# bede/kindel

Measured on NVIDIA H100. Metric: aligned bases/sec through pileup+consensus, higher is better.
Workload: dtype int32

## Files before the change

kindel_b200/csrc/api.cu:

```cuda
#include <atomic>
#include <cstdio>
#include <cstdlib>
#include <cstring>
#include <new>

#include "kdl_common.cuh"
#include "pileup_general.cu"
#include "pileup_simple.cu"
#include "pileup_tile.cu"
#include "pileup_mask.cu"
#include "vote.cu"
#include "assemble.cu"
#include "variants.cu"
#include "select.cu"
#include "primers.cu"
#include "mates.cu"
#include "quality.cu"
#include "amplicons.cu"
#include "normalise.cu"

namespace {

std::atomic<long long> g_launches{0};

inline int grid_for(long long items, int per_block, int cap) {
    long long g = (items + per_block - 1) / per_block;
    if (g < 1) g = 1;
    if (g > cap) g = cap;
    return (int)g;
}

#ifndef KDL_HOST_EMU
constexpr int kMaxDevices = 64;

inline int current_device() {
    int dev = 0;
    if (cudaGetDevice(&dev) != cudaSuccess || dev < 0 || dev >= kMaxDevices) dev = 0;
    return dev;
}

inline int sm_count() {
    static std::atomic<int> cache[kMaxDevices];
    const int dev = current_device();
    int n = cache[dev].load(std::memory_order_relaxed);
    if (n <= 0) {
        if (cudaDeviceGetAttribute(&n, cudaDevAttrMultiProcessorCount, dev) != cudaSuccess || n <= 0) n = 132;
        cache[dev].store(n, std::memory_order_relaxed);
    }
    return n;
}

template <int kFlush, bool kCx>
inline int ensure_tile_smem() {
    static std::atomic<int> done[kMaxDevices];
    const int dev = current_device();
    if (done[dev].load(std::memory_order_acquire)) return KDL_OK;
    if (cudaFuncSetAttribute(kdl::pileup_tile_kernel<kFlush, kCx>, cudaFuncAttributeMaxDynamicSharedMemorySize,
                             (int)sizeof(kdl::TileSmem<kdl::TileCfg<kCx>>)) != cudaSuccess)
        return KDL_ERR_CUDA;
    done[dev].store(1, std::memory_order_release);
    return KDL_OK;
}

inline int check_launch() {
    g_launches.fetch_add(1, std::memory_order_relaxed);
    return cudaGetLastError() == cudaSuccess ? KDL_OK : KDL_ERR_CUDA;
}
#else
inline int sm_count() { return emu::M().sm_count; }

template <int kFlush, bool kCx>
inline int ensure_tile_smem() { return KDL_OK; }

inline int check_launch() {
    g_launches.fetch_add(1, std::memory_order_relaxed);
    return emu::take_launch_error() ? KDL_ERR_CUDA : KDL_OK;
}
#endif

template <int kFlush, bool kCx>
inline int launch_tile(const kdl_batch& b, int32_t* counts, long long n_slots, long long tile_lo, long long n_tiles,
                       int split, int zero_rest, uint32_t* dirty_map, uint32_t map_after, cudaStream_t st) {
    int rc = ensure_tile_smem<kFlush, kCx>();
    if (rc != KDL_OK) return rc;
    const long long units = n_tiles * split, max_grid = (long long)sm_count() * 2;
    const long long grid = units < max_grid ? units : max_grid;
    KDL_LAUNCH((kdl::pileup_tile_kernel<kFlush, kCx>), (unsigned)grid, kdl::W_THREADS,
               sizeof(kdl::TileSmem<kdl::TileCfg<kCx>>), st,
               b, counts, n_slots, b.tile_index, tile_lo, n_tiles, split, zero_rest, dirty_map, map_after);
    return KDL_OK;
}

int validate_batch(const kdl_batch* b) {
    if (!b || b->n_reads < 0 || b->n_contigs < 0 || b->n_hard < 0 || b->n_complex < b->n_hard)
        return KDL_ERR_INVALID_ARG;
    if (b->n_reads > 0 && (!b->ref_start || !b->seq_off || !b->l_seq || !b->seq4 ||
                           !b->contig_read_off || !b->contig_len || !b->contig_slot))
        return KDL_ERR_INVALID_ARG;
    if ((b->n_hard > 0 && !b->hard_idx) || (b->n_complex > 0 && !b->complex_idx)) return KDL_ERR_INVALID_ARG;
    if (b->reach_right < b->max_simple_len || b->reach_left < 0) return KDL_ERR_INVALID_ARG;
    return KDL_OK;
}

}

extern "C" {

int kdl_abi_version(void) { return KDL_ABI_VERSION; }

const char* kdl_status_string(int status) {
    switch (status) {
        case KDL_OK: return "ok";
        case KDL_ERR_INVALID_ARG: return "invalid argument";
        case KDL_ERR_CUDA: return "CUDA error";
        case KDL_ERR_NO_DEVICE: return "no CUDA device";
        case KDL_ERR_INDEX: return "IndexError: read walks off the contig or off its SEQ";
        case KDL_ERR_KEY: return "KeyError: base outside A,C,G,T,N in an M or S op";
        default: return "unknown status";
    }
}

int64_t kdl_launch_count(void) { return g_launches.load(std::memory_order_relaxed); }

int kdl_pileup(const kdl_batch* batch, int32_t* counts, int64_t n_slots, int32_t* ins_events,
               int32_t* err_flag, void* stream) {
    return kdl_pileup_range(batch, counts, n_slots, 0, n_slots, 0, ins_events, err_flag, stream);
}

int kdl_pileup_range(const kdl_batch* batch, int32_t* counts, int64_t n_slots, int64_t slot_lo,
                     int64_t slot_hi, int32_t flags, int32_t* ins_events, int32_t* err_flag, void* stream) {
    return kdl_pileup_range_map(batch, counts, n_slots, slot_lo, slot_hi, flags, nullptr, ins_events, err_flag, stream);
}

int kdl_pileup_range_map(const kdl_batch* batch, int32_t* counts, int64_t n_slots, int64_t slot_lo, int64_t slot_hi,
                         int32_t flags, uint32_t* dirty_map, int32_t* ins_events, int32_t* err_flag, void* stream) {
    int rc = validate_batch(batch);
    if (rc != KDL_OK) return rc;
    if (!counts || !err_flag || n_slots <= 0 || slot_lo < 0 || slot_hi > n_slots || slot_lo > slot_hi ||
        (reinterpret_cast<uintptr_t>(dirty_map) & 15))
        return KDL_ERR_INVALID_ARG;
    const bool tileable = (n_slots % KDL_TILE) == 0 && (slot_lo % KDL_TILE) == 0 && (slot_hi % KDL_TILE) == 0;
    if ((slot_lo & 3) || (slot_hi & 3)) return KDL_ERR_INVALID_ARG;
    cudaStream_t st = (cudaStream_t)stream;
    const int cap = sm_count() * 8;
    const bool has_tile_reads = batch->n_reads > batch->n_hard;
    const bool tiled = has_tile_reads && tileable && batch->reads_sorted && batch->tile_index &&
                       batch->reach_right > 0 && batch->reach_right <= KDL_FAST_MAXLEN + KDL_TILE_MAXREACH;
    const bool fresh = (flags & KDL_PILEUP_FRESH_WEIGHTS) != 0;
    const long long tile_lo = slot_lo / KDL_TILE, n_tiles = (slot_hi - slot_lo) / KDL_TILE;
    int split = 1;
    if (tiled && n_tiles > 0) {
        const long long slots = (long long)sm_count() * 2;
        if (n_tiles < slots) {
            long long want = (slots + n_tiles - 1) / n_tiles;
            const long long deep = batch->n_reads / (n_tiles * 256);
            if (want > deep) want = deep;
            split = (int)(want < 1 ? 1 : (want > 32 ? 32 : want));
        }
        if (const char* ev = getenv("KDL_SPLIT")) { const int v = atoi(ev); if (v >= 1 && v <= 64) split = v; }
    }
    bool cx_by_atomics = (batch->n_complex - batch->n_hard) * 16 < batch->n_reads;
    if (const char* ev = getenv("KDL_CX")) cx_by_atomics = !strcmp(ev, "atomics") ? true : (!strcmp(ev, "pieces") ? false : cx_by_atomics);
    const int zero_in_k1 = (tiled && split == 1 && fresh && n_tiles > 0 && (flags & KDL_PILEUP_ZERO_REST)) ? 1 : 0;
    const int zero_from = (fresh && !(tiled && split == 1)) ? 0 : 5;
    const int zero_to = ((flags & KDL_PILEUP_ZERO_REST) && !zero_in_k1) ? KDL_NCOL : 5;
    const bool zero_pass = zero_to > zero_from && slot_hi > slot_lo;
    const bool k1_stores = tiled && split == 1 && fresh && n_tiles > 0;
    const bool saturate = dirty_map && batch->n_complex > 0 && batch->n_complex * 16 >= batch->n_reads &&
                          (k1_stores || zero_pass);
    uint32_t* mark_map = saturate ? nullptr : dirty_map;
    if (zero_pass) {
        uint32_t* zmap = saturate || (zero_from <= 5 && zero_to == KDL_NCOL) ? dirty_map : nullptr;
        KDL_LAUNCH(kdl::zero_cols_kernel, sm_count() * 4, 256, 0, st, counts, n_slots, zero_from, zero_to, slot_lo,
                   slot_hi, zmap, saturate ? ~0u : 0u);
        if ((rc = check_launch()) != KDL_OK) return rc;
    }
    const uint32_t map_after = saturate && k1_stores ? ~0u : 0u;
    if (batch->n_reads == 0) return KDL_OK;
    if (tiled) {
        if (n_tiles > 0) {
            KDL_LAUNCH(kdl::tile_index_kernel, (unsigned)((n_tiles * 32 + 255) / 256), 256, 0, st, *batch, tile_lo,
                       n_tiles, batch->tile_index);
            if ((rc = check_launch()) != KDL_OK) return rc;
            const bool cx = batch->n_complex > batch->n_hard && !cx_by_atomics;
            if (split > 1) {
                rc = cx ? launch_tile<kdl::F_ATOMIC, true>(*batch, counts, n_slots, tile_lo, n_tiles, split, 0, nullptr, 0, st)
                        : launch_tile<kdl::F_ATOMIC, false>(*batch, counts, n_slots, tile_lo, n_tiles, split, 0, nullptr, 0, st);
            } else if (fresh) {
                rc = cx ? launch_tile<kdl::F_STORE, true>(*batch, counts, n_slots, tile_lo, n_tiles, 1, zero_in_k1, dirty_map,
                                                          map_after, st)
                        : launch_tile<kdl::F_STORE, false>(*batch, counts, n_slots, tile_lo, n_tiles, 1, zero_in_k1, dirty_map,
                                                           map_after, st);
            } else {
                rc = cx ? launch_tile<kdl::F_ADD, true>(*batch, counts, n_slots, tile_lo, n_tiles, 1, 0, nullptr, 0, st)
                        : launch_tile<kdl::F_ADD, false>(*batch, counts, n_slots, tile_lo, n_tiles, 1, 0, nullptr, 0, st);
            }
            if (rc != KDL_OK) return rc;
            if ((rc = check_launch()) != KDL_OK) return rc;
        }
        if (batch->n_complex > batch->n_hard) {
            if (cx_by_atomics)
                KDL_LAUNCH(kdl::pileup_events_kernel<8>, (unsigned)((batch->n_complex + 31) / 32), 256, 0, st,
                           *batch, counts, n_slots, ins_events, 1, mark_map);
            else
                KDL_LAUNCH(kdl::pileup_events_kernel<1>, (unsigned)((batch->n_complex + 255) / 256), 256, 0, st,
                           *batch, counts, n_slots, ins_events, 0, mark_map);
            if ((rc = check_launch()) != KDL_OK) return rc;
        }
        if (batch->n_hard > 0) {
            const int grid = grid_for(batch->n_hard, 8, cap);
            KDL_LAUNCH(kdl::pileup_general_kernel, grid, 256, 0, st, *batch, batch->hard_idx, batch->n_hard, counts,
                       n_slots, ins_events, err_flag, mark_map);
            if ((rc = check_launch()) != KDL_OK) return rc;
        }
    } else {
        if (batch->n_reads > batch->n_complex) {
            const int grid = grid_for(batch->n_reads, 8, cap);
            KDL_LAUNCH(kdl::pileup_simple_atomic_kernel, grid, 256, 0, st, *batch, counts, n_slots, err_flag);
            if ((rc = check_launch()) != KDL_OK) return rc;
        }
        if (batch->n_complex > 0) {
            const int grid = grid_for(batch->n_reads, 8, cap);
            KDL_LAUNCH(kdl::pileup_general_kernel, grid, 256, 0, st, *batch, nullptr, batch->n_reads, counts, n_slots,
                       ins_events, err_flag, mark_map);
            if ((rc = check_launch()) != KDL_OK) return rc;
        }
    }
    return KDL_OK;
}

int kdl_unmask(const kdl_batch* batch, const kdl_qmask* qmask, int32_t* counts, int64_t n_slots, void* stream) {
    int rc = validate_batch(batch);
    if (rc != KDL_OK) return rc;
    if (!qmask || !counts || n_slots <= 0 || qmask->n_reads < 0 || qmask->n_bases < 0 || qmask->n_reads > batch->n_reads)
        return KDL_ERR_INVALID_ARG;
    if (qmask->n_reads == 0) return KDL_OK;
    if (!qmask->read_idx || !qmask->off || !qmask->qpos) return KDL_ERR_INVALID_ARG;
    const long long grid = (qmask->n_reads + kdl::kQThreads - 1) / kdl::kQThreads;
    KDL_LAUNCH(kdl::unmask_kernel, (unsigned)grid, kdl::kQThreads, 0, (cudaStream_t)stream, *batch, *qmask, counts,
               n_slots);
    return check_launch();
}

int kdl_diagnose(const kdl_batch* batch, kdl_diag* diag_dev, void* stream) {
    int rc = validate_batch(batch);
    if (rc != KDL_OK) return rc;
    if (!diag_dev) return KDL_ERR_INVALID_ARG;
    cudaStream_t st = (cudaStream_t)stream;
    KDL_LAUNCH(kdl::diagnose_init_kernel, 1, 1, 0, st, diag_dev);
    if ((rc = check_launch()) != KDL_OK) return rc;
    if (batch->n_hard > 0) {
        const long long grid = (batch->n_hard + 255) / 256;
        KDL_LAUNCH(kdl::diagnose_kernel, (unsigned)grid, 256, 0, st, *batch, diag_dev);
        if ((rc = check_launch()) != KDL_OK) return rc;
    }
    KDL_LAUNCH(kdl::diagnose_final_kernel, 1, 1, 0, st, diag_dev);
    return check_launch();
}

int kdl_vote(const int32_t* counts, int64_t n_slots, int64_t min_depth_ceil, uint8_t* calls,
             void* stream) {
    if (!counts || !calls || n_slots <= 0 || (n_slots & 3)) return KDL_ERR_INVALID_ARG;
    kdl::Peers none;
    none.n = 0;
    const long long quads = n_slots / 4;
    const long long grid = (quads + 255) / 256;
    KDL_LAUNCH(kdl::vote_kernel<false>, (unsigned)grid, 256, 0, (cudaStream_t)stream,
               counts, none, n_slots, 0, n_slots, min_depth_ceil, calls, nullptr, kdl::MajorityVote{});
    return check_launch();
}

static bool valid_threshold(double t) { return t >= 0.0 && t <= 1.0; }

int kdl_vote_iupac(const int32_t* counts, int64_t n_slots, int64_t min_depth_ceil, double threshold, uint8_t* calls,
                   void* stream) {
    if (!counts || !calls || n_slots <= 0 || (n_slots & 3) || !valid_threshold(threshold)) return KDL_ERR_INVALID_ARG;
    kdl::Peers none;
    none.n = 0;
    const long long quads = n_slots / 4;
    const long long grid = (quads + 255) / 256;
    KDL_LAUNCH((kdl::vote_kernel<false, kdl::IupacVote>), (unsigned)grid, 256, 0, (cudaStream_t)stream,
               counts, none, n_slots, 0, n_slots, min_depth_ceil, calls, nullptr, kdl::IupacVote{threshold});
    return check_launch();
}

int kdl_derive(const int32_t* counts, int64_t n_slots, int32_t* out, void* stream) {
    if (!counts || !out || n_slots <= 0) return KDL_ERR_INVALID_ARG;
    const long long grid = (n_slots + 255) / 256;
    KDL_LAUNCH(kdl::derive_kernel, (unsigned)grid, 256, 0, (cudaStream_t)stream, counts, n_slots, out);
    return check_launch();
}

int kdl_vote_peers(const int32_t* const* peer_counts, int32_t n_peers, int64_t n_slots,
                   int64_t slot_lo, int64_t slot_hi, int64_t min_depth_ceil, uint8_t* calls,
                   int32_t* reduced, void* stream) {
    return kdl_vote_peers_sparse(peer_counts, nullptr, nullptr, n_peers, n_slots, slot_lo, slot_hi,
                                 min_depth_ceil, calls, reduced, stream);
}

static int make_exchange(const kdl_exchange* x, kdl::Exchange* e, int64_t n_slots) {
    if (!x || x->n_ranks < 1 || x->n_ranks > 16 || x->rank < 0 || x->rank >= x->n_ranks || !x->counter)
        return KDL_ERR_INVALID_ARG;
    e->peers.n = x->n_ranks;
    e->rank = x->rank;
    e->counter = x->counter;
    for (int p = 0; p < x->n_ranks; ++p) {
        if (!x->tables[p] || !x->calls[p] || !x->ready[p] || !x->done[p]) return KDL_ERR_INVALID_ARG;
        e->peers.tab[p] = x->tables[p];
        e->peers.lo[p] = x->foot_lo[p];
        e->peers.hi[p] = n_slots > 0 && x->foot_hi[p] > n_slots ? n_slots : x->foot_hi[p];
        if ((e->peers.lo[p] & 3) || (e->peers.hi[p] & 3)) return KDL_ERR_INVALID_ARG;
        e->calls[p] = x->calls[p];
        e->ready[p] = x->ready[p];
        e->done[p] = x->done[p];
        e->slice_lo[p] = x->slice_lo[p];
        e->slice_hi[p] = x->slice_hi[p];
        if ((x->slice_lo[p] & 3) || (x->slice_hi[p] & 3) || x->slice_hi[p] < x->slice_lo[p]) return KDL_ERR_INVALID_ARG;
    }
    e->ready_local = x->ready[x->rank];
    e->done_local = x->done[x->rank];
    return KDL_OK;
}

int kdl_exchange_signal(const kdl_exchange* x, int32_t epoch, void* stream) {
    kdl::Exchange e;
    int rc = make_exchange(x, &e, 0);
    if (rc != KDL_OK) return rc;
    KDL_LAUNCH(kdl::exchange_signal_kernel, 1, 32, 0, (cudaStream_t)stream, e, epoch);
    return check_launch();
}

int kdl_exchange_wait(const kdl_exchange* x, int32_t epoch, void* stream) {
    kdl::Exchange e;
    int rc = make_exchange(x, &e, 0);
    if (rc != KDL_OK) return rc;
    dim3 grid((unsigned)(sm_count() * 2 / x->n_ranks + 1), (unsigned)x->n_ranks);
    KDL_LAUNCH(kdl::exchange_gather_kernel, grid, 256, 0, (cudaStream_t)stream, e, epoch);
    return check_launch();
}

extern "C++" template <class Vote>
int exchange_vote(const kdl_exchange* x, int64_t n_slots, int64_t min_depth_ceil, int32_t epoch, Vote vote,
                  void* stream) {
    if (n_slots <= 0 || (n_slots & 3)) return KDL_ERR_INVALID_ARG;
    kdl::Exchange e;
    int rc = make_exchange(x, &e, n_slots);
    if (rc != KDL_OK) return rc;
    if (x->slice_hi[x->rank] > n_slots) return KDL_ERR_INVALID_ARG;
    const long long quads = (x->slice_hi[x->rank] - x->slice_lo[x->rank]) / 4;
    long long grid = (quads + 255) / 256;
    const long long cap = (long long)sm_count() * 8;
    if (grid > cap) grid = cap;
    if (grid < 1) grid = 1;
    KDL_LAUNCH(kdl::vote_exchange_kernel<Vote>, (unsigned)grid, 256, 0, (cudaStream_t)stream, e, n_slots,
               min_depth_ceil, epoch, vote);
    return check_launch();
}

int kdl_exchange_vote(const kdl_exchange* x, int64_t n_slots, int64_t min_depth_ceil, int32_t epoch,
                      void* stream) {
    return exchange_vote(x, n_slots, min_depth_ceil, epoch, kdl::MajorityVote{}, stream);
}

int kdl_exchange_vote_iupac(const kdl_exchange* x, int64_t n_slots, int64_t min_depth_ceil, double threshold,
                            int32_t epoch, void* stream) {
    if (!valid_threshold(threshold)) return KDL_ERR_INVALID_ARG;
    return exchange_vote(x, n_slots, min_depth_ceil, epoch, kdl::IupacVote{threshold}, stream);
}

int kdl_cdr_flags(const int32_t* counts, int64_t n_slots, int64_t slot_lo, int64_t slot_hi,
                  double clip_decay_threshold, uint8_t* flags, uint8_t* bases, void* stream) {
    if (!counts || !flags || !bases || n_slots <= 0 || slot_lo < 0 || slot_hi > n_slots || slot_lo > slot_hi)
        return KDL_ERR_INVALID_ARG;
    if (slot_hi == slot_lo) return KDL_OK;
    const long long grid = (slot_hi - slot_lo + 255) / 256;
    KDL_LAUNCH(kdl::cdr_flags_kernel, (unsigned)grid, 256, 0, (cudaStream_t)stream, counts, n_slots, slot_lo, slot_hi,
               clip_decay_threshold, flags, bases);
    return check_launch();
}

int64_t kdl_assemble_scratch_words(int64_t n_slots) {
    return n_slots < 0 ? 0 : (n_slots + 1 + kdl::A_BLOCK - 1) / kdl::A_BLOCK + 1;
}

int kdl_assemble(const uint8_t* calls, int64_t n_slots, const int64_t* contig_slot, const int32_t* contig_len,
                 int32_t n_contigs, const int64_t* ins_slot, const uint32_t* ins_off, const uint8_t* ins_bytes,
                 int64_t n_ins, uint32_t* block_sums, uint32_t* offsets, uint8_t* out, void* stream) {
    if (!calls || n_slots <= 0 || !contig_slot || !contig_len || n_contigs < 0 || n_ins < 0 || !block_sums || !offsets ||
        !out || (n_ins > 0 && (!ins_slot || !ins_off || !ins_bytes)))
        return KDL_ERR_INVALID_ARG;
    kdl::AssembleArgs a;
    a.calls = calls; a.n_slots = n_slots; a.contig_slot = contig_slot; a.contig_len = contig_len; a.n_contigs = n_contigs;
    a.ins_slot = ins_slot; a.ins_off = ins_off; a.ins_bytes = ins_bytes; a.n_ins = n_ins;
    const long long n_blocks = (n_slots + 1 + kdl::A_BLOCK - 1) / kdl::A_BLOCK;
    cudaStream_t st = (cudaStream_t)stream;
    int rc;
    KDL_LAUNCH(kdl::assemble_sums_kernel, (unsigned)n_blocks, kdl::A_THREADS, 0, st, a, block_sums);
    if ((rc = check_launch()) != KDL_OK) return rc;
    KDL_LAUNCH(kdl::assemble_scan_sums_kernel, 1, kdl::A_THREADS, 0, st, block_sums, n_blocks);
    if ((rc = check_launch()) != KDL_OK) return rc;
    KDL_LAUNCH(kdl::assemble_scatter_kernel, (unsigned)n_blocks, kdl::A_THREADS, 0, st, a, block_sums, offsets, out);
    return check_launch();
}

int kdl_consensus_qual(const int32_t* counts, const uint8_t* calls, int64_t n_slots, uint8_t* qual, void* stream) {
    if (!counts || !calls || !qual || n_slots <= 0 || (n_slots & 3)) return KDL_ERR_INVALID_ARG;
    const long long grid = (n_slots / 4 + 255) / 256;
    KDL_LAUNCH(kdl::consensus_qual_kernel, (unsigned)grid, 256, 0, (cudaStream_t)stream, counts, calls, n_slots, qual);
    return check_launch();
}

int kdl_assemble_qual(const uint32_t* offsets, const uint8_t* qual, int64_t n_slots, const int64_t* ins_slot,
                      const uint8_t* ins_qual, int64_t n_ins, uint8_t* out, void* stream) {
    if (!offsets || !qual || !out || n_slots <= 0 || n_ins < 0 || (n_ins > 0 && (!ins_slot || !ins_qual)))
        return KDL_ERR_INVALID_ARG;
    const long long n_blocks = (n_slots + kdl::A_BLOCK - 1) / kdl::A_BLOCK;
    KDL_LAUNCH(kdl::assemble_qual_kernel, (unsigned)n_blocks, kdl::A_THREADS, 0, (cudaStream_t)stream,
               offsets, qual, n_slots, ins_slot, ins_qual, n_ins, out);
    return check_launch();
}

int64_t kdl_variant_scratch_words(int64_t n_slots) {
    return n_slots < 0 ? 0 : (n_slots + kdl::A_BLOCK - 1) / kdl::A_BLOCK + 1;
}

static int variant_args(const int32_t* counts, int64_t n_slots, const int64_t* contig_slot, const int32_t* contig_len,
                        int32_t n_contigs, int64_t abs_floor, double rel_threshold, kdl::VariantArgs* a) {
    if (!counts || n_slots <= 0 || (n_slots & 3) || n_slots > (int64_t)UINT32_MAX || n_contigs < 0 ||
        (n_contigs > 0 && (!contig_slot || !contig_len)) || abs_floor < -1 || abs_floor > (1LL << 31))
        return KDL_ERR_INVALID_ARG;
    *a = kdl::VariantArgs{};
    a->counts = counts; a->n_slots = n_slots;
    a->layout.contig_slot = contig_slot; a->layout.contig_len = contig_len; a->layout.n_contigs = n_contigs;
    a->abs_floor = abs_floor; a->rel_threshold = rel_threshold;
    return KDL_OK;
}

int kdl_variant_count(const int32_t* counts, int64_t n_slots, const int64_t* contig_slot, const int32_t* contig_len,
                      int32_t n_contigs, int64_t abs_floor, double rel_threshold, uint32_t* block_sums, void* stream) {
    kdl::VariantArgs a;
    int rc = variant_args(counts, n_slots, contig_slot, contig_len, n_contigs, abs_floor, rel_threshold, &a);
    if (rc != KDL_OK) return rc;
    if (!block_sums) return KDL_ERR_INVALID_ARG;
    const long long n_blocks = (n_slots + kdl::A_BLOCK - 1) / kdl::A_BLOCK;
    cudaStream_t st = (cudaStream_t)stream;
    KDL_LAUNCH(kdl::variant_sums_kernel, (unsigned)n_blocks, kdl::A_THREADS, 0, st, a, block_sums);
    if ((rc = check_launch()) != KDL_OK) return rc;
    KDL_LAUNCH(kdl::assemble_scan_sums_kernel, 1, kdl::A_THREADS, 0, st, block_sums, n_blocks);
    return check_launch();
}

int kdl_variant_scatter(const int32_t* counts, int64_t n_slots, const int64_t* contig_slot, const int32_t* contig_len,
                        int32_t n_contigs, int64_t abs_floor, double rel_threshold, const uint32_t* block_sums,
                        int64_t n_sites, int64_t* site_slot, int32_t* site_counts, uint8_t* site_mask, void* stream) {
    kdl::VariantArgs a;
    int rc = variant_args(counts, n_slots, contig_slot, contig_len, n_contigs, abs_floor, rel_threshold, &a);
    if (rc != KDL_OK) return rc;
    if (!block_sums || n_sites < 0 || n_sites > n_slots || (n_sites > 0 && (!site_slot || !site_counts || !site_mask)))
        return KDL_ERR_INVALID_ARG;
    const long long n_blocks = (n_slots + kdl::A_BLOCK - 1) / kdl::A_BLOCK;
    KDL_LAUNCH(kdl::variant_scatter_kernel, (unsigned)n_blocks, kdl::A_THREADS, 0, (cudaStream_t)stream,
               a, block_sums, n_sites, site_slot, site_counts, site_mask);
    return check_launch();
}

static int variant_ref_args(const int32_t* counts, int64_t n_slots, const int64_t* contig_slot,
                            const int32_t* contig_len, int32_t n_contigs, const uint8_t* ref, int64_t abs_floor,
                            double rel_threshold, kdl::RefVariantArgs* a) {
    kdl::VariantArgs v;
    int rc = variant_args(counts, n_slots, contig_slot, contig_len, n_contigs, abs_floor, rel_threshold, &v);
    if (rc != KDL_OK) return rc;
    if (!ref || (reinterpret_cast<uintptr_t>(ref) & 3)) return KDL_ERR_INVALID_ARG;
    *a = kdl::RefVariantArgs{};
    a->counts = counts; a->n_slots = n_slots; a->layout = v.layout; a->ref = ref;
    a->abs_floor = abs_floor; a->rel_threshold = rel_threshold;
    return KDL_OK;
}

int kdl_variant_ref_count(const int32_t* counts, int64_t n_slots, const int64_t* contig_slot, const int32_t* contig_len,
                          int32_t n_contigs, const uint8_t* ref, int64_t abs_floor, double rel_threshold,
                          uint32_t* block_sums, void* stream) {
    kdl::RefVariantArgs a;
    int rc = variant_ref_args(counts, n_slots, contig_slot, contig_len, n_contigs, ref, abs_floor, rel_threshold, &a);
    if (rc != KDL_OK) return rc;
    if (!block_sums) return KDL_ERR_INVALID_ARG;
    const long long n_blocks = (n_slots + kdl::A_BLOCK - 1) / kdl::A_BLOCK;
    cudaStream_t st = (cudaStream_t)stream;
    KDL_LAUNCH(kdl::variant_ref_sums_kernel, (unsigned)n_blocks, kdl::A_THREADS, 0, st, a, block_sums);
    if ((rc = check_launch()) != KDL_OK) return rc;
    KDL_LAUNCH(kdl::assemble_scan_sums_kernel, 1, kdl::A_THREADS, 0, st, block_sums, n_blocks);
    return check_launch();
}

int kdl_variant_ref_scatter(const int32_t* counts, int64_t n_slots, const int64_t* contig_slot,
                            const int32_t* contig_len, int32_t n_contigs, const uint8_t* ref, int64_t abs_floor,
                            double rel_threshold, const uint32_t* block_sums, int64_t n_sites, int64_t* site_slot,
                            int32_t* site_counts, int64_t* site_dpa, uint8_t* site_mask, void* stream) {
    kdl::RefVariantArgs a;
    int rc = variant_ref_args(counts, n_slots, contig_slot, contig_len, n_contigs, ref, abs_floor, rel_threshold, &a);
    if (rc != KDL_OK) return rc;
    if (!block_sums || n_sites < 0 || n_sites > n_slots ||
        (n_sites > 0 && (!site_slot || !site_counts || !site_dpa || !site_mask)))
        return KDL_ERR_INVALID_ARG;
    const long long n_blocks = (n_slots + kdl::A_BLOCK - 1) / kdl::A_BLOCK;
    KDL_LAUNCH(kdl::variant_ref_scatter_kernel, (unsigned)n_blocks, kdl::A_THREADS, 0, (cudaStream_t)stream,
               a, block_sums, n_sites, site_slot, site_counts, site_dpa, site_mask);
    return check_launch();
}

// ... 446 lines not shown
```

kindel_b200/csrc/pileup_general.cu:

```cuda
#include "kdl_common.cuh"

namespace kdl {

__global__ void __launch_bounds__(256)
pileup_general_kernel(kdl_batch b, const uint32_t* __restrict__ list, long long n_list, int32_t* __restrict__ counts,
                      long long n_slots, int32_t* __restrict__ ins_events, int32_t* __restrict__ err_flag,
                      uint32_t* __restrict__ dirty_map = nullptr) {
    const int lane = threadIdx.x & 31;
    const bool marks = dirty_map != nullptr && lane == 0;
    const long long warp0 = ((long long)blockIdx.x * blockDim.x + threadIdx.x) >> 5;
    const long long n_warps = ((long long)gridDim.x * blockDim.x) >> 5;
    bool bad = false;

    for (long long j = warp0; j < n_list; j += n_warps) {
        const long long r = list ? (long long)list[j] : j;
        const uint32_t lraw = (uint32_t)b.l_seq[r];
        if (!(lraw & KDL_COMPLEX)) continue;
        const int c = find_contig(b.contig_read_off, b.n_contigs, r);
        const long long L = b.contig_len[c];
        const long long base = b.contig_slot[c];
        const long long lseq = complex_len(lraw);
        const uint32_t* __restrict__ seq = b.seq4 + (size_t)b.seq_off[r];
        const uint32_t* __restrict__ blk = seq + ((lseq + 7) >> 3);
        const uint32_t c0 = 0, c1 = blk[0];
        const uint32_t* __restrict__ cig = blk + 2;
        long long r_pos = b.ref_start[r];
        long long q_pos = 0;
        uint32_t evt = blk[1];

        for (uint32_t i = c0; i < c1; ++i) {
            const uint32_t cg = cig[i];
            const long long len = cg >> 4;
            const int op = cg & 0xF;
            if (op == 0 || op == 7 || op == 8) {
                for (long long k = lane; k < len; k += 32) {
                    const long long q = q_pos + k;
                    const long long idx = pyindex(r_pos + k, L);
                    if (q >= lseq || idx < 0) { bad = true; continue; }
                    const int col = nib2col(nibble_at(seq, q));
                    if (col < 0) { bad = true; continue; }
                    atomicAdd(counts + (long long)(KDL_W_A + col) * n_slots + base + idx, 1);
                }
                r_pos += len;
                q_pos += len;
            } else if (op == 1) {
                if (marks) mark_dirty_py(dirty_map, KDL_INS, 1, base, r_pos, r_pos + 1, L + 1);
                if (lane == 0) {
                    const long long idx = pyindex(r_pos, L + 1);
                    if (idx < 0) {
                        bad = true;
                    } else {
                        atomicAdd(counts + (long long)KDL_INS * n_slots + base + idx, 1);
                        if (ins_events) {
                            int4 e = make_int4((int)(base + idx), (int)r, (int)q_pos, (int)len);
                            reinterpret_cast<int4*>(ins_events)[evt] = e;
                        }
                    }
                }
                evt += 1;
                q_pos += len;
            } else if (op == 2) {
                if (marks) mark_dirty_py(dirty_map, KDL_DEL, 1, base, r_pos, r_pos + len, L + 1);
                for (long long k = lane; k < len; k += 32) {
                    const long long idx = pyindex(r_pos + k, L + 1);
                    if (idx < 0) { bad = true; continue; }
                    atomicAdd(counts + (long long)KDL_DEL * n_slots + base + idx, 1);
                }
                r_pos += len;
            } else if (op == 4) {
                if (i == c0) {
                    if (marks) {
                        mark_dirty_py(dirty_map, KDL_CLIP_ENDS, 1, base, r_pos, r_pos + 1, L + 1);
                        mark_dirty(dirty_map, KDL_CEW_A, 5, base + (r_pos - len > 0 ? r_pos - len : 0),
                                   base + (r_pos < L ? r_pos : L));
                    }
                    if (lane == 0) {
                        const long long idx = pyindex(r_pos, L + 1);
                        if (idx < 0) bad = true;
                        else atomicAdd(counts + (long long)KDL_CLIP_ENDS * n_slots + base + idx, 1);
                    }
                    for (long long g = lane; g < len; g += 32) {
                        if (g >= lseq) { bad = true; continue; }
                        const long long rel = r_pos - len + g;
                        if (rel < 0) continue;
                        if (rel >= L) { bad = true; continue; }
                        const int col = nib2col(nibble_at(seq, g));
                        if (col < 0) { bad = true; continue; }
                        atomicAdd(counts + (long long)(KDL_CEW_A + col) * n_slots + base + rel, 1);
                    }
                    q_pos += len;
                } else {
                    if (lane == 0) {
                        const long long idx = pyindex(r_pos - 1, L + 1);
                        if (idx < 0) bad = true;
                        else atomicAdd(counts + (long long)KDL_CLIP_STARTS * n_slots + base + idx, 1);
                    }
                    long long n_adv = L - r_pos;
                    n_adv = n_adv < 0 ? 0 : (n_adv > len ? len : n_adv);
                    if (marks) {
                        mark_dirty_py(dirty_map, KDL_CLIP_STARTS, 1, base, r_pos - 1, r_pos, L + 1);
                        mark_dirty_py(dirty_map, KDL_CSW_A, 5, base, r_pos, r_pos + n_adv, L);
                    }
                    for (long long k = lane; k < n_adv; k += 32) {
                        const long long q = q_pos + k;
                        const long long idx = pyindex(r_pos + k, L);
                        if (q >= lseq || idx < 0) { bad = true; continue; }
                        const int col = nib2col(nibble_at(seq, q));
                        if (col < 0) { bad = true; continue; }
                        atomicAdd(counts + (long long)(KDL_CSW_A + col) * n_slots + base + idx, 1);
                    }
                    if (n_adv < len && q_pos + n_adv >= lseq) bad = true;
                    r_pos += n_adv;
                    q_pos += n_adv;
                }
            }
        }
    }
    if (bad) atomicOr(err_flag, 1);
}

template <int kLanes>
__global__ void __launch_bounds__(256)
pileup_events_kernel(kdl_batch b, int32_t* __restrict__ counts, long long n_slots, int32_t* __restrict__ ins_events,
                     int with_m, uint32_t* __restrict__ dirty_map = nullptr) {
    const int lane = (int)(threadIdx.x % kLanes);
    constexpr int kStep = kLanes;
    const long long gtid = (long long)blockIdx.x * blockDim.x + threadIdx.x;
    const long long j = gtid / kLanes;
    if (j >= b.n_complex) return;
    const long long r = (long long)b.complex_idx[j];
    const uint32_t lraw = (uint32_t)b.l_seq[r];
    if ((lraw & (KDL_COMPLEX | KDL_HARD)) != KDL_COMPLEX) return;
    const int c = find_contig(b.contig_read_off, b.n_contigs, r);
    const long long slot0 = b.contig_slot[c];
    int32_t* __restrict__ tab = counts + slot0;
    const uint32_t* __restrict__ seq = b.seq4 + (size_t)b.seq_off[r];
    const uint32_t* __restrict__ blk = seq + (((lraw & KDL_LEN_MASK) + 7) >> 3);
    const int n_ops = (int)blk[0];
    uint32_t evt = blk[1];
    const uint32_t* __restrict__ ops = blk + 2;
    long long r_pos = b.ref_start[r];
    int q_pos = 0;
    const bool marks = dirty_map != nullptr && lane == 0;
    for (int o = 0; o < n_ops; ++o) {
        const uint32_t cg = ops[o];
        const int len = (int)(cg >> 4);
        const int op = (int)(cg & 0xF);
        if (op == 0 || op == 7 || op == 8) {
            if (with_m)
                for (int d = lane; d < len; d += kStep)
                    atomicAdd(tab + (long long)(KDL_W_A + nib2col(nibble_at(seq, q_pos + d))) * n_slots + r_pos + d, 1);
            r_pos += len;
            q_pos += len;
        } else if (op == 1) {
            if (lane == 0) {
                if (marks) mark_dirty(dirty_map, KDL_INS, 1, slot0 + r_pos, slot0 + r_pos + 1);
                atomicAdd(tab + (long long)KDL_INS * n_slots + r_pos, 1);
                if (ins_events)
                    reinterpret_cast<int4*>(ins_events)[evt] = make_int4((int)(slot0 + r_pos), (int)r, q_pos, len);
            }
            evt += 1;
            q_pos += len;
        } else if (op == 2) {
            if (marks) mark_dirty(dirty_map, KDL_DEL, 1, slot0 + r_pos, slot0 + r_pos + len);
            for (int d = lane; d < len; d += kStep) atomicAdd(tab + (long long)KDL_DEL * n_slots + r_pos + d, 1);
            r_pos += len;
        } else if (op == 4) {
            if (o == 0) {
                if (marks) {
                    mark_dirty(dirty_map, KDL_CLIP_ENDS, 1, slot0 + r_pos, slot0 + r_pos + 1);
                    mark_dirty(dirty_map, KDL_CEW_A, 5, slot0 + (r_pos - len > 0 ? r_pos - len : 0), slot0 + r_pos);
                }
                if (lane == 0) atomicAdd(tab + (long long)KDL_CLIP_ENDS * n_slots + r_pos, 1);
                for (int g = lane; g < len; g += kStep) {
                    const long long rel = r_pos - len + g;
                    if (rel >= 0) atomicAdd(tab + (long long)(KDL_CEW_A + nib2col(nibble_at(seq, g))) * n_slots + rel, 1);
                }
                q_pos += len;
            } else {
                if (marks) {
                    mark_dirty(dirty_map, KDL_CLIP_STARTS, 1, slot0 + r_pos - 1, slot0 + r_pos);
                    mark_dirty(dirty_map, KDL_CSW_A, 5, slot0 + r_pos, slot0 + r_pos + len);
                }
                if (lane == 0) atomicAdd(tab + (long long)KDL_CLIP_STARTS * n_slots + r_pos - 1, 1);
                for (int d = lane; d < len; d += kStep)
                    atomicAdd(tab + (long long)(KDL_CSW_A + nib2col(nibble_at(seq, q_pos + d))) * n_slots + r_pos + d, 1);
                r_pos += len;
                q_pos += len;
            }
        }
    }
}

__device__ unsigned long long diagnose_read(const kdl_batch& b, long long j) {
    const long long r = (long long)b.hard_idx[j];
    const int c = find_contig(b.contig_read_off, b.n_contigs, r);
    const long long L = b.contig_len[c];
    const long long lseq = complex_len((uint32_t)b.l_seq[r]);
    const uint32_t* __restrict__ seq = b.seq4 + (size_t)b.seq_off[r];
    const uint32_t* __restrict__ blk = seq + ((lseq + 7) >> 3);
    const uint32_t c0 = 0, c1 = blk[0];
    const uint32_t* __restrict__ cig = blk + 2;
    long long r_pos = b.ref_start[r], q_pos = 0;
#define KDL_FAIL(kind, nib)                                                                     \
    return ((unsigned long long)r << 24) | ((unsigned long long)(kind) << 20) |                 \
           ((unsigned long long)(nib) << 16) | (unsigned long long)((i - c0) > 0xFFFF ? 0xFFFF : (i - c0))
    for (uint32_t i = c0; i < c1; ++i) {
        const uint32_t cg = cig[i];
        const long long len = cg >> 4;
        const int op = cg & 0xF;
        if (op == 0 || op == 7 || op == 8) {
            for (long long k = 0; k < len; ++k) {
                if (q_pos >= lseq) KDL_FAIL(0, 0);
                if (pyindex(r_pos, L) < 0) KDL_FAIL(0, 0);
                const int nib = nibble_at(seq, q_pos);
                if (nib2col(nib) < 0) KDL_FAIL(1, nib);
                ++r_pos; ++q_pos;
            }
        } else if (op == 1) {
            if (pyindex(r_pos, L + 1) < 0) KDL_FAIL(0, 0);
            q_pos += len;
        } else if (op == 2) {
            for (long long k = 0; k < len; ++k)
                if (pyindex(r_pos + k, L + 1) < 0) KDL_FAIL(0, 0);
            r_pos += len;
        } else if (op == 4) {
            if (i == c0) {
                if (pyindex(r_pos, L + 1) < 0) KDL_FAIL(0, 0);
                for (long long g = 0; g < len; ++g) {
                    if (g >= lseq) KDL_FAIL(0, 0);
                    const long long rel = r_pos - len + g;
                    if (rel >= 0) {
                        if (rel >= L) KDL_FAIL(0, 0);
                        const int nib = nibble_at(seq, g);
                        if (nib2col(nib) < 0) KDL_FAIL(1, nib);
                    }
                }
                q_pos += len;
            } else {
                if (pyindex(r_pos - 1, L + 1) < 0) KDL_FAIL(0, 0);
                for (long long k = 0; k < len; ++k) {
                    if (q_pos >= lseq) KDL_FAIL(0, 0);
                    if (r_pos < L) {
                        if (pyindex(r_pos, L) < 0) KDL_FAIL(0, 0);
                        const int nib = nibble_at(seq, q_pos);
                        if (nib2col(nib) < 0) KDL_FAIL(1, nib);
                        ++r_pos; ++q_pos;
                    }
                }
            }
        }
    }
#undef KDL_FAIL
    return ~0ull;
}

__global__ void diagnose_init_kernel(kdl_diag* d) {
    d->status = 0; d->reserved = 0; d->read = -1; d->nibble = 0; d->op_index = 0;
    *reinterpret_cast<unsigned long long*>(&d->read) = ~0ull;
}

__global__ void __launch_bounds__(256) diagnose_kernel(kdl_batch b, kdl_diag* d) {
    const long long j = (long long)blockIdx.x * blockDim.x + threadIdx.x;
    if (j >= b.n_hard) return;
    const unsigned long long key = diagnose_read(b, j);
    if (key != ~0ull) atomicMin(reinterpret_cast<unsigned long long*>(&d->read), key);
}

__global__ void diagnose_final_kernel(kdl_diag* d) {
    const unsigned long long key = *reinterpret_cast<unsigned long long*>(&d->read);
    if (key == ~0ull) { d->status = KDL_OK; d->read = -1; return; }
    d->status = ((key >> 20) & 0xF) ? KDL_ERR_KEY : KDL_ERR_INDEX;
    d->nibble = (int)((key >> 16) & 0xF);
    d->op_index = (int)(key & 0xFFFF);
    d->read = (long long)(key >> 24);
}

}
```

Before: 1777 billion.

## Accumulate complex-read pileup per slot window in shared memory

Replaces the global-atomic events kernel for complex reads with a window kernel. Each block owns a 1024-slot window, finds its complex reads with a warp-cooperative binary search, accumulates match/ins/del counts into shared memory, and then flushes them to global memory with vector adds, or with atomics when the window is split. This cuts global atomic traffic and contention. The events kernel becomes single-thread-per-read and no longer handles matches. The trade-off is an extra search, per-window shared-memory zeroing, and duplicated work for reads that span windows.

```diff
diff --git a/kindel_b200/csrc/api.cu b/kindel_b200/csrc/api.cu
--- a/kindel_b200/csrc/api.cu
+++ b/kindel_b200/csrc/api.cu
@@ -91,6 +91,19 @@
     return KDL_OK;
 }
 
+int depth_split(long long units, int per_sm, long long reads) {
+    int split = 1;
+    const long long slots = (long long)sm_count() * per_sm;
+    if (units < slots) {
+        long long want = (slots + units - 1) / units;
+        const long long deep = reads / (units * 256);
+        if (want > deep) want = deep;
+        split = (int)(want < 1 ? 1 : (want > 32 ? 32 : want));
+    }
+    if (const char* ev = getenv("KDL_SPLIT")) { const int v = atoi(ev); if (v >= 1 && v <= 64) split = v; }
+    return split;
+}
+
 int validate_batch(const kdl_batch* b) {
     if (!b || b->n_reads < 0 || b->n_contigs < 0 || b->n_hard < 0 || b->n_complex < b->n_hard)
         return KDL_ERR_INVALID_ARG;
@@ -148,17 +161,7 @@
                        batch->reach_right > 0 && batch->reach_right <= KDL_FAST_MAXLEN + KDL_TILE_MAXREACH;
     const bool fresh = (flags & KDL_PILEUP_FRESH_WEIGHTS) != 0;
     const long long tile_lo = slot_lo / KDL_TILE, n_tiles = (slot_hi - slot_lo) / KDL_TILE;
-    int split = 1;
-    if (tiled && n_tiles > 0) {
-        const long long slots = (long long)sm_count() * 2;
-        if (n_tiles < slots) {
-            long long want = (slots + n_tiles - 1) / n_tiles;
-            const long long deep = batch->n_reads / (n_tiles * 256);
-            if (want > deep) want = deep;
-            split = (int)(want < 1 ? 1 : (want > 32 ? 32 : want));
-        }
-        if (const char* ev = getenv("KDL_SPLIT")) { const int v = atoi(ev); if (v >= 1 && v <= 64) split = v; }
-    }
+    const int split = tiled && n_tiles > 0 ? depth_split(n_tiles, 2, batch->n_reads) : 1;
     bool cx_by_atomics = (batch->n_complex - batch->n_hard) * 16 < batch->n_reads;
     if (const char* ev = getenv("KDL_CX")) cx_by_atomics = !strcmp(ev, "atomics") ? true : (!strcmp(ev, "pieces") ? false : cx_by_atomics);
     const int zero_in_k1 = (tiled && split == 1 && fresh && n_tiles > 0 && (flags & KDL_PILEUP_ZERO_REST)) ? 1 : 0;
@@ -198,13 +201,16 @@
             if (rc != KDL_OK) return rc;
             if ((rc = check_launch()) != KDL_OK) return rc;
         }
-        if (batch->n_complex > batch->n_hard) {
-            if (cx_by_atomics)
-                KDL_LAUNCH(kdl::pileup_events_kernel<8>, (unsigned)((batch->n_complex + 31) / 32), 256, 0, st,
-                           *batch, counts, n_slots, ins_events, 1, mark_map);
-            else
-                KDL_LAUNCH(kdl::pileup_events_kernel<1>, (unsigned)((batch->n_complex + 255) / 256), 256, 0, st,
-                           *batch, counts, n_slots, ins_events, 0, mark_map);
+        if (batch->n_complex > batch->n_hard && cx_by_atomics && n_tiles > 0) {
+            const long long n_win = (slot_hi - slot_lo + kdl::CW_SLOTS - 1) / kdl::CW_SLOTS;
+            const int wsplit = depth_split(n_win, 8, batch->n_complex - batch->n_hard);
+            KDL_LAUNCH(kdl::pileup_window_kernel, (unsigned)(n_win * wsplit), kdl::CW_THREADS,
+                       sizeof(int32_t) * kdl::CW_SMEM_COLS * kdl::CW_SLOTS, st, *batch, counts, n_slots, slot_lo,
+                       slot_hi, wsplit, ins_events, mark_map);
+            if ((rc = check_launch()) != KDL_OK) return rc;
+        } else if (batch->n_complex > batch->n_hard && !cx_by_atomics) {
+            KDL_LAUNCH(kdl::pileup_events_kernel, (unsigned)((batch->n_complex + 255) / 256), 256, 0, st, *batch, counts,
+                       n_slots, ins_events, mark_map);
             if ((rc = check_launch()) != KDL_OK) return rc;
         }
         if (batch->n_hard > 0) {
diff --git a/kindel_b200/csrc/pileup_general.cu b/kindel_b200/csrc/pileup_general.cu
--- a/kindel_b200/csrc/pileup_general.cu
+++ b/kindel_b200/csrc/pileup_general.cu
@@ -1,4 +1,4 @@
-#include "kdl_common.cuh"
+#include "tile_common.cuh"
 
 namespace kdl {
 
@@ -119,14 +119,10 @@
     if (bad) atomicOr(err_flag, 1);
 }
 
-template <int kLanes>
 __global__ void __launch_bounds__(256)
 pileup_events_kernel(kdl_batch b, int32_t* __restrict__ counts, long long n_slots, int32_t* __restrict__ ins_events,
-                     int with_m, uint32_t* __restrict__ dirty_map = nullptr) {
-    const int lane = (int)(threadIdx.x % kLanes);
-    constexpr int kStep = kLanes;
-    const long long gtid = (long long)blockIdx.x * blockDim.x + threadIdx.x;
-    const long long j = gtid / kLanes;
+                     uint32_t* __restrict__ dirty_map) {
+    const long long j = (long long)blockIdx.x * blockDim.x + threadIdx.x;
     if (j >= b.n_complex) return;
     const long long r = (long long)b.complex_idx[j];
     const uint32_t lraw = (uint32_t)b.l_seq[r];
@@ -141,53 +137,202 @@
     const uint32_t* __restrict__ ops = blk + 2;
     long long r_pos = b.ref_start[r];
     int q_pos = 0;
-    const bool marks = dirty_map != nullptr && lane == 0;
     for (int o = 0; o < n_ops; ++o) {
         const uint32_t cg = ops[o];
         const int len = (int)(cg >> 4);
         const int op = (int)(cg & 0xF);
         if (op == 0 || op == 7 || op == 8) {
-            if (with_m)
-                for (int d = lane; d < len; d += kStep)
-                    atomicAdd(tab + (long long)(KDL_W_A + nib2col(nibble_at(seq, q_pos + d))) * n_slots + r_pos + d, 1);
             r_pos += len;
             q_pos += len;
         } else if (op == 1) {
-            if (lane == 0) {
-                if (marks) mark_dirty(dirty_map, KDL_INS, 1, slot0 + r_pos, slot0 + r_pos + 1);
-                atomicAdd(tab + (long long)KDL_INS * n_slots + r_pos, 1);
-                if (ins_events)
-                    reinterpret_cast<int4*>(ins_events)[evt] = make_int4((int)(slot0 + r_pos), (int)r, q_pos, len);
-            }
+            if (dirty_map) mark_dirty(dirty_map, KDL_INS, 1, slot0 + r_pos, slot0 + r_pos + 1);
+            atomicAdd(tab + (long long)KDL_INS * n_slots + r_pos, 1);
+            if (ins_events)
+                reinterpret_cast<int4*>(ins_events)[evt] = make_int4((int)(slot0 + r_pos), (int)r, q_pos, len);
             evt += 1;
             q_pos += len;
         } else if (op == 2) {
-            if (marks) mark_dirty(dirty_map, KDL_DEL, 1, slot0 + r_pos, slot0 + r_pos + len);
-            for (int d = lane; d < len; d += kStep) atomicAdd(tab + (long long)KDL_DEL * n_slots + r_pos + d, 1);
+            if (dirty_map) mark_dirty(dirty_map, KDL_DEL, 1, slot0 + r_pos, slot0 + r_pos + len);
+            for (int d = 0; d < len; ++d) atomicAdd(tab + (long long)KDL_DEL * n_slots + r_pos + d, 1);
             r_pos += len;
         } else if (op == 4) {
             if (o == 0) {
-                if (marks) {
+                if (dirty_map) {
                     mark_dirty(dirty_map, KDL_CLIP_ENDS, 1, slot0 + r_pos, slot0 + r_pos + 1);
                     mark_dirty(dirty_map, KDL_CEW_A, 5, slot0 + (r_pos - len > 0 ? r_pos - len : 0), slot0 + r_pos);
                 }
-                if (lane == 0) atomicAdd(tab + (long long)KDL_CLIP_ENDS * n_slots + r_pos, 1);
-                for (int g = lane; g < len; g += kStep) {
+                atomicAdd(tab + (long long)KDL_CLIP_ENDS * n_slots + r_pos, 1);
+                for (int g = 0; g < len; ++g) {
                     const long long rel = r_pos - len + g;
                     if (rel >= 0) atomicAdd(tab + (long long)(KDL_CEW_A + nib2col(nibble_at(seq, g))) * n_slots + rel, 1);
                 }
                 q_pos += len;
             } else {
-                if (marks) {
+                if (dirty_map) {
                     mark_dirty(dirty_map, KDL_CLIP_STARTS, 1, slot0 + r_pos - 1, slot0 + r_pos);
                     mark_dirty(dirty_map, KDL_CSW_A, 5, slot0 + r_pos, slot0 + r_pos + len);
                 }
-                if (lane == 0) atomicAdd(tab + (long long)KDL_CLIP_STARTS * n_slots + r_pos - 1, 1);
-                for (int d = lane; d < len; d += kStep)
+                atomicAdd(tab + (long long)KDL_CLIP_STARTS * n_slots + r_pos - 1, 1);
+                for (int d = 0; d < len; ++d)
                     atomicAdd(tab + (long long)(KDL_CSW_A + nib2col(nibble_at(seq, q_pos + d))) * n_slots + r_pos + d, 1);
                 r_pos += len;
                 q_pos += len;
             }
+        }
+    }
+}
+
+constexpr int CW_SLOTS = 1024;
+constexpr int CW_THREADS = 256;
+constexpr int CW_SMEM_COLS = 7;
+static_assert(CW_SLOTS % KDL_TILE == 0 && CW_SLOTS % 256 == 0, "windows of whole tiles, whole map records per warp");
+
+__device__ __forceinline__ void lower_bound2_u32(const uint32_t* __restrict__ a, long long n, uint32_t key1,
+                                                 uint32_t key2, int lane, long long& r1, long long& r2) {
+    long long lo[2] = {0, 0}, hi[2] = {n, n};
+    const uint32_t key[2] = {key1, key2};
+    while (lo[0] < hi[0] || lo[1] < hi[1]) {
+        long long step[2];
+        bool ge[2];
+#pragma unroll
+        for (int k = 0; k < 2; ++k) {
+            step[k] = (hi[k] - lo[k] + 31) >> 5;
+            const long long i = lo[k] + (long long)(lane + 1) * step[k] - 1;
+            ge[k] = lo[k] >= hi[k] || i >= hi[k] || a[i] >= key[k];
+        }
+#pragma unroll
+        for (int k = 0; k < 2; ++k) {
+            const unsigned m = __ballot_sync(0xffffffffu, ge[k]);
+            if (lo[k] >= hi[k]) continue;
+            if (m == 0u) { lo[k] = hi[k]; continue; }
+            const int b = __ffs(m) - 1;
+            const long long nl = lo[k] + (long long)b * step[k], nh = nl + step[k] - 1;
+            hi[k] = nh < hi[k] ? nh : hi[k];
+            lo[k] = step[k] == 1 ? hi[k] : nl;
+        }
+    }
+    r1 = lo[0];
+    r2 = lo[1];
+}
+
+__global__ void __launch_bounds__(CW_THREADS)
+pileup_window_kernel(kdl_batch b, int32_t* __restrict__ counts, long long n_slots, long long slot_lo, long long slot_hi,
+                     int split, int32_t* __restrict__ ins_events, uint32_t* __restrict__ dirty_map) {
+    KDL_DYNAMIC_SMEM(smem_raw);
+    int* acc = reinterpret_cast<int*>(smem_raw);
+    __shared__ long long range[2];
+    const int tid = threadIdx.x, lane = tid & 31;
+    constexpr int n_sec = CW_SMEM_COLS * (CW_SLOTS / 8);
+    const long long g0 = slot_lo + (long long)(blockIdx.x / split) * CW_SLOTS;
+    const long long g1 = g0 + CW_SLOTS < slot_hi ? g0 + CW_SLOTS : slot_hi;
+    for (int k = tid; k < 2 * n_sec; k += CW_THREADS) reinterpret_cast<int4*>(acc)[k] = make_int4(0, 0, 0, 0);
+    if (tid < 32) {
+        const uint32_t lo = b.tile_index[F_IDX * (g0 / KDL_TILE)], hi = b.tile_index[F_IDX * ((g1 - 1) / KDL_TILE) + 1];
+        long long ja, je;
+        lower_bound2_u32(b.complex_idx, b.n_complex, lo, hi, lane, ja, je);
+        if (lane == 0) {
+            const int part = (int)(blockIdx.x % split);
+            range[0] = ja + (je - ja) * part / split;
+            range[1] = ja + (je - ja) * (part + 1) / split;
+        }
+    }
+    __syncthreads();
+    const long long j0 = range[0], j1 = range[1];
+    int lg = 0;
+    while (lg < 5 && ((j1 - j0) << (lg + 1)) <= CW_THREADS) ++lg;
+    const int gl = tid & ((1 << lg) - 1), step = 1 << lg;
+    for (long long j = j0 + (tid >> lg); j < j1; j += CW_THREADS >> lg) {
+        const long long r = (long long)b.complex_idx[j];
+        const uint32_t lraw = (uint32_t)b.l_seq[r];
+        if ((lraw & (KDL_COMPLEX | KDL_HARD)) != KDL_COMPLEX) continue;
+        const int c = find_contig(b.contig_read_off, b.n_contigs, r);
+        const long long slot0 = b.contig_slot[c];
+        const long long wl = g0 - slot0, wh = g1 - slot0;
+        int32_t* __restrict__ tab = counts + slot0;
+        const uint32_t* __restrict__ seq = b.seq4 + (size_t)b.seq_off[r];
+        const uint32_t* __restrict__ blk = seq + (((lraw & KDL_LEN_MASK) + 7) >> 3);
+        const int n_ops = (int)blk[0];
+        uint32_t evt = blk[1];
+        const uint32_t* __restrict__ ops = blk + 2;
+        long long r_pos = b.ref_start[r];
+        int q_pos = 0;
+        const bool marks = dirty_map != nullptr && gl == 0;
+        for (int o = 0; o < n_ops; ++o) {
+            const uint32_t cg = ops[o];
+            const int len = (int)(cg >> 4);
+            const int op = (int)(cg & 0xF);
+            const long long s0 = r_pos > wl ? r_pos : wl, s1 = r_pos + len < wh ? r_pos + len : wh;
+            if (op == 0 || op == 7 || op == 8) {
+#pragma unroll 4
+                for (long long s = s0 + gl; s < s1; s += step)
+                    atomicAdd(acc + (KDL_W_A + nib2col(nibble_at(seq, q_pos + (s - r_pos)))) * CW_SLOTS + (s - wl), 1);
+                r_pos += len;
+                q_pos += len;
+            } else if (op == 1) {
+                if (gl == 0 && r_pos >= wl && r_pos < wh) {
+                    atomicAdd(acc + KDL_INS * CW_SLOTS + (r_pos - wl), 1);
+                    if (ins_events)
+                        reinterpret_cast<int4*>(ins_events)[evt] = make_int4((int)(slot0 + r_pos), (int)r, q_pos, len);
+                }
+                evt += 1;
+                q_pos += len;
+            } else if (op == 2) {
+                for (long long s = s0 + gl; s < s1; s += step) atomicAdd(acc + KDL_DEL * CW_SLOTS + (s - wl), 1);
+                r_pos += len;
+            } else if (op == 4) {
+                if (o == 0) {
+                    const long long e0 = r_pos - len, c1 = r_pos < wh ? r_pos : wh;
+                    long long c0 = e0 > 0 ? e0 : 0;
+                    if (c0 < wl) c0 = wl;
+                    if (gl == 0 && r_pos >= wl && r_pos < wh) {
+                        if (marks) mark_dirty(dirty_map, KDL_CLIP_ENDS, 1, slot0 + r_pos, slot0 + r_pos + 1);
+                        atomicAdd(tab + (long long)KDL_CLIP_ENDS * n_slots + r_pos, 1);
+                    }
+                    if (marks) mark_dirty(dirty_map, KDL_CEW_A, 5, slot0 + c0, slot0 + c1);
+                    for (long long s = c0 + gl; s < c1; s += step)
+                        atomicAdd(tab + (long long)(KDL_CEW_A + nib2col(nibble_at(seq, s - e0))) * n_slots + s, 1);
+                    q_pos += len;
+                } else {
+                    if (gl == 0 && r_pos - 1 >= wl && r_pos - 1 < wh) {
+                        if (marks) mark_dirty(dirty_map, KDL_CLIP_STARTS, 1, slot0 + r_pos - 1, slot0 + r_pos);
+                        atomicAdd(tab + (long long)KDL_CLIP_STARTS * n_slots + r_pos - 1, 1);
+                    }
+                    if (marks) mark_dirty(dirty_map, KDL_CSW_A, 5, slot0 + s0, slot0 + s1);
+                    for (long long s = s0 + gl; s < s1; s += step)
+                        atomicAdd(tab + (long long)(KDL_CSW_A + nib2col(nibble_at(seq, q_pos + (s - r_pos)))) * n_slots + s,
+                                  1);
+                    r_pos += len;
+                    q_pos += len;
+                }
+            }
+        }
+    }
+    __syncthreads();
+    for (int sec = tid; sec < n_sec; sec += CW_THREADS) {
+        const int col = sec / (CW_SLOTS / 8), off = 8 * (sec % (CW_SLOTS / 8));
+        const int4* sp = reinterpret_cast<const int4*>(acc) + 2 * sec;
+        const int4 d0 = sp[0], d1 = sp[1];
+        const bool dirty = (d0.x | d0.y | d0.z | d0.w | d1.x | d1.y | d1.z | d1.w) != 0;
+        int32_t* dst = counts + (long long)col * n_slots + g0 + off;
+        if (dirty && split == 1) {
+            int4* p = reinterpret_cast<int4*>(dst);
+            int4 v0 = p[0], v1 = p[1];
+            v0.x += d0.x; v0.y += d0.y; v0.z += d0.z; v0.w += d0.w;
+            v1.x += d1.x; v1.y += d1.y; v1.z += d1.z; v1.w += d1.w;
+            p[0] = v0;
+            p[1] = v1;
+        } else if (dirty) {
+            const int d[8] = {d0.x, d0.y, d0.z, d0.w, d1.x, d1.y, d1.z, d1.w};
+#pragma unroll
+            for (int k = 0; k < 8; ++k)
+                if (d[k]) atomicAdd(dst + k, d[k]);
+        }
+        if (dirty_map && col >= KDL_DEL) {
+            const unsigned m = __ballot_sync(0xffffffffu, dirty);
+            const unsigned bits = lane < 4 ? (m >> (8 * lane)) & 0xFFu : 0u;
+            if (bits)
+                atomicOr(dirty_map + 4 * ((g0 + off - 8 * lane) / 64 + lane) + (col - KDL_DEL) / 4,
+                         bits << (8 * ((col - KDL_DEL) % 4)));
         }
     }
 }
```

Measured after the change: 1899 billion, median of 6. 1.07x the previous value.
